# jcmgray/cotengra

Hardware: NVIDIA H100
Metric: sycamore_n53_m20_sliced_contract_tflops (higher is better)
Workload: dtype c128 (f64 arithmetic)

## Files before the change

### cotengra_b200/_lib.py

```python

from __future__ import annotations

import ctypes as C
import os

from . import lowering

_HERE = os.path.dirname(os.path.abspath(__file__))
LIB_PATH = os.path.join(_HERE, "libctgb200.so")

EXPORTS = (
    "ctgb_abi_version",
    "ctgb_desc_words",
    "ctgb_single_desc_words",
    "ctgb_last_error",
    "ctgb_device_info",
    "ctgb_contract_pair",
    "ctgb_reduce_single",
    "ctgb_plan_create",
    "ctgb_plan_set_chunk_desc",
    "ctgb_plan_set_scale_slots",
    "ctgb_plan_set_accumulator",
    "ctgb_plan_destroy",
    "ctgb_plan_workspace_bytes",
    "ctgb_plan_launches_per_slice",
    "ctgb_plan_strip_modes",
    "ctgb_plan_execute",
    "ctgb_plan_execute_host",
    "ctgb_launch_count",
    "ctgb_tensor_map_launches",
    "ctgb_plan_profile",
    "ctgb_plan_profile_read",
    "ctgb_probe_fp64_peaks",
    "ctgb_tc05_launch_config",
    "ctgb_dmmastream_launch_config",
)
TC05_LAUNCH_FIELDS = ("b_stat", "nb", "sa", "grid", "smem", "tm_rank", "bulk", "chunk_steps", "chunks")
DMMASTREAM_LAUNCH_FIELDS = ("nj", "rows", "grid")


class CtgbTensor(C.Structure):
    _fields_ = [
        ("kind", C.c_int32),
        ("input_index", C.c_int32),
        ("offset", C.c_int64),
        ("nbytes", C.c_int64),
        ("n_sliced", C.c_int32),
        ("slice_pos", C.POINTER(C.c_int32)),
        ("slice_stride", C.POINTER(C.c_int64)),
    ]
# ... 52 lines not shown
        if not hasattr(lib, name):
            raise ImportError(f"{LIB_PATH} does not export {name}")
    lib.ctgb_last_error.restype = C.c_char_p
    lib.ctgb_launch_count.restype = C.c_int64
    lib.ctgb_tensor_map_launches.restype = C.c_int64
    lib.ctgb_plan_workspace_bytes.restype = C.c_size_t
    lib.ctgb_plan_workspace_bytes.argtypes = [C.c_void_p]
    lib.ctgb_plan_launches_per_slice.restype = C.c_int64
    lib.ctgb_plan_launches_per_slice.argtypes = [C.c_void_p]
    lib.ctgb_plan_strip_modes.argtypes = [C.c_void_p, C.POINTER(C.c_int32), C.POINTER(C.c_int32), C.c_int]
    lib.ctgb_device_info.argtypes = [
        C.POINTER(C.c_int), C.POINTER(C.c_int), C.POINTER(C.c_int), C.POINTER(C.c_size_t)
    ]
    lib.ctgb_contract_pair.argtypes = [C.c_void_p] * 5
    lib.ctgb_reduce_single.argtypes = [C.c_void_p] * 4
    lib.ctgb_plan_create.argtypes = [C.POINTER(CtgbPlanDesc), C.POINTER(C.c_void_p)]
    lib.ctgb_plan_set_chunk_desc.argtypes = [C.c_void_p, C.c_void_p]
    lib.ctgb_plan_set_scale_slots.argtypes = [C.c_void_p, C.POINTER(C.c_int32), C.POINTER(C.c_int32), C.c_int]
    lib.ctgb_plan_set_accumulator.argtypes = [C.c_void_p, C.c_int32]
    lib.ctgb_plan_destroy.argtypes = [C.c_void_p]
    lib.ctgb_plan_destroy.restype = None
    lib.ctgb_plan_execute.argtypes = [
        C.c_void_p, C.POINTER(C.c_void_p), C.c_void_p, C.c_void_p, C.c_void_p, C.POINTER(C.c_void_p),
        C.c_void_p, C.c_size_t, C.c_int64, C.c_int64, C.c_int64, C.c_void_p,
    ]
    lib.ctgb_plan_execute_host.argtypes = [
        C.c_void_p, C.POINTER(C.c_void_p), C.POINTER(C.c_int64), C.c_void_p,
        C.POINTER(C.c_double), C.c_void_p, C.c_size_t, C.c_int64, C.c_int64,
        C.c_int64, C.c_void_p,
    ]
# ... 62 lines not shown
```

### cotengra_b200/contract.py

```python

from __future__ import annotations

import ctypes as C
import functools
import math
import warnings

import numpy as np

from . import _lib, lowering
from .executor import ExecPlan, output_chunking
from .lowering import (
    build_pair_desc,
    build_single_desc,
    check_accumulate,
    check_precision,
    check_tensordot_shapes,
    classify_pair,
    classify_single,
    dtype_name,
    split_equation,
    tensordot_terms,
)
from .tree import TreeSpec
# ... 110 lines not shown
    ta, tb, to = tensordot_terms(axes, na, nb)
    return _run_pair(ta, a, tb, b, to, precision)


def implementation(precision="3xtf32"):
    if check_precision(precision) == "3xtf32":
        return (einsum, tensordot)
    return (functools.partial(einsum, precision=precision), functools.partial(tensordot, precision=precision))




class _Executor:

    def __init__(self, contractions, inputs, output, size_dict, sliced, dtype, strip_exponent=False, device=None,
                 vjp_max_bytes=None, precision="3xtf32", stripped_grad=False, accumulate="native", **plan_opts):
        torch = _torch()
        self._ir, self._plan_opts = contractions, plan_opts
        self._program, self._sliced = (contractions, inputs, output, size_dict), sliced
        self.device = torch.device("cuda", torch.cuda.current_device() if device is None else device)
        with torch.cuda.device(self.device):
            self.plan = ExecPlan(*self._program, sliced, dtype=dtype, strip_exponent=strip_exponent,
                                 precision=precision, accumulate=accumulate, **plan_opts).create()
        self.dtype = self.plan.dtype
        self.precision = precision
        self.accumulate = accumulate
        self.out_dtype = self.plan.acc_dtype
        self.strip_exponent = bool(strip_exponent)
        self.stripped_grad = bool(stripped_grad)
        self.vjp_max_bytes = vjp_max_bytes
        self._shapes = [tuple(size_dict[ix] for ix in term) for term in inputs]
        self._ws = None
        self._vjp_plans, self._vjp_ws = {}, None

    @property
    def nslices(self):
        return self.plan.nslices

# ... 120 lines not shown
    def __init__(self, tree, dtype="complex128", strip_exponent=False, device=None,
                 contractions=None, fuse=True, vjp_max_bytes=None, precision="3xtf32", stripped_grad=False,
                 accumulate="native", **plan_opts):
        check_precision(precision, dtype)
        check_accumulate(accumulate)
        self.spec = spec = tree if isinstance(tree, TreeSpec) else TreeSpec.from_cotengra(tree)
        self.exec_spec, self.fusion = spec, {"changed": False}
        if fuse and contractions is None:
            from .fusion import fuse_stems

            opts = fuse if isinstance(fuse, dict) else {}
            self.exec_spec, self.fusion = fuse_stems(spec, dtype_name(dtype), **opts)
        ir = self.exec_spec.contractions() if contractions is None else contractions
        super().__init__(ir, spec.inputs, spec.output, spec.size_dict, spec.sliced, dtype,
                         strip_exponent=strip_exponent, device=device, vjp_max_bytes=vjp_max_bytes,
                         precision=precision, stripped_grad=stripped_grad, accumulate=accumulate, **plan_opts)
        self._ref_work = None

    @property
    def reference_work(self):
        if self._ref_work is None:
            if self.fusion.get("changed"):
                from .fusion import tree_work

                self._ref_work = tree_work(self.spec)
            else:
                self._ref_work = (self.plan.macs_per_slice, self.plan.macs_invariant,
                                  self.plan.elements_per_slice)
        return self._ref_work

    def __call__(self, arrays, **kw):
# ... 411 lines not shown
```

### cotengra_b200/csrc/ctg_b200.cu

```cuda
#include <cuda.h>
#include <cuda_runtime.h>
#include <stdint.h>
#include <stdio.h>
#include <stdlib.h>
#include <string.h>

#include <algorithm>
#include <atomic>
#include <type_traits>
#include <string>
#include <vector>

#include "../../include/ctg_b200.h"
#include "gett_desc.h"
#include "gett_kernels.cuh"
#include "probe.cuh"

using namespace ctgb;

namespace {

thread_local std::string g_err;
std::atomic<int64_t> g_launches{0};

// ... 237 lines not shown
  const bool strip = desc_stripped(h);
  const double2 *a = (const double2*)A, *b = (const double2*)B;
  double2* c = (double2*)C;
  const unsigned blocks = (unsigned)lc.blocks;
  switch (lc.nj) {
    case 1: dmmastream_launch<1, 4>(strip, blocks, d, a, b, c, st); break;
    case 2: dmmastream_launch<2, 4>(strip, blocks, d, a, b, c, st); break;
    case 4: dmmastream_launch<4, 4>(strip, blocks, d, a, b, c, st); break;
    default: dmmastream_launch<8, 2>(strip, blocks, d, a, b, c, st); break;
  }
  g_launches.fetch_add(1, std::memory_order_relaxed);
  CUDA_TRY(cudaGetLastError());
  return CTGB_OK;
}

std::atomic<int64_t> g_tmap_launches{0};

struct Tc05Box {
  int nb = 0;
  struct Dim { uint64_t ext, stride; } dim[8];
};
int tc05_tensor_map_box(const int64_t* h, uint64_t a_addr, Tc05Box& bx) {
  if (a_addr & 15u) return 0;
  auto& box = bx.dim;
  int& nb = bx.nb;
  nb = 0;
  const int n_lda = (int)h[W_NLDA];
  for (int i = 0; i < n_lda; ++i) {
    const uint64_t ext = (uint64_t)h[OFF_LDA + 4 * i], st = (uint64_t)h[OFF_LDA + 4 * i + 1];
    if (h[OFF_LDA + 4 * i + 1] <= 0) return 0;
// ... 236 lines not shown
             : launch_gett_policy<T, Tf32Policy<T, __VA_ARGS__>>(h, d, A, B, C, st)
      case VAR_DMMA_128x64: CTGB_TF32(4, 2, 2, 4, 16, 3);
      case VAR_DMMA_64x128: CTGB_TF32(2, 4, 2, 4, 16, 3);
      case VAR_DMMA_256x32: CTGB_TF32(8, 1, 2, 4, 8, 3);
      case VAR_DMMA_256x16: CTGB_TF32(8, 1, 2, 2, 8, 3);
      case VAR_TF32_32x32: CTGB_TF32(2, 2, 1, 2, 16, 4);
#undef CTGB_TF32
      default: break;
    }
  }
  return fail(CTGB_E_VALUE, "unknown kernel variant for this dtype");
}

int launch_gett(const int64_t* h, const int64_t* d, const void* A, const void* B, void* C, cudaStream_t st) {
  if (h[W_MAGIC] != DESC_MAGIC) return fail(CTGB_E_VALUE, "bad pair descriptor magic");
  switch ((int)h[W_DTYPE]) {
    case CTGB_F32: return launch_gett_typed<float>(h, d, A, B, C, st);
    case CTGB_F64: return launch_gett_typed<double>(h, d, A, B, C, st);
    case CTGB_C64: return launch_gett_typed<float2>(h, d, A, B, C, st);
    case CTGB_C128: return launch_gett_typed<double2>(h, d, A, B, C, st);
  }
  return fail(CTGB_E_VALUE, "bad dtype");
}

template <typename T>
int launch_single_typed(const int64_t* h, const int64_t* d, const void* X, void* out, cudaStream_t st) {
  long long n = h[S_OUT_ELEMS];
  if (n <= 0) return CTGB_OK;
  const long long cap = (long long)(devinfo().ok ? devinfo().sms : 132) * 16;
  long long blocks = (n + 255) / 256;
// ... 373 lines not shown
  cudaFree(sink);
  return rc;
}

int ctgb_contract_pair(const int64_t* desc, const void* A, const void* B, void* C, void* stream) {
  if (!desc) return fail(CTGB_E_VALUE, "null descriptor");
  cudaStream_t st = (cudaStream_t)stream;
  int64_t* d = nullptr;
  CUDA_TRY(cudaMallocAsync((void**)&d, DESC_WORDS * sizeof(int64_t), st));
  CUDA_TRY(cudaMemcpyAsync(d, desc, DESC_WORDS * sizeof(int64_t), cudaMemcpyHostToDevice, st));
  int rc = launch_gett(desc, d, A, B, C, st);
  cudaFreeAsync(d, st);
  return rc;
}

int ctgb_reduce_single(const int64_t* desc, const void* X, void* out, void* stream) {
  if (!desc) return fail(CTGB_E_VALUE, "null descriptor");
  cudaStream_t st = (cudaStream_t)stream;
  int64_t* d = nullptr;
  CUDA_TRY(cudaMallocAsync((void**)&d, SDESC_WORDS * sizeof(int64_t), st));
  CUDA_TRY(cudaMemcpyAsync(d, desc, SDESC_WORDS * sizeof(int64_t), cudaMemcpyHostToDevice, st));
  int rc = launch_single(desc, d, X, out, st);
  cudaFreeAsync(d, st);
  return rc;
}

int ctgb_plan_create(const ctgb_plan_desc* pd, ctgb_plan** out) {
  if (!pd || !out) return fail(CTGB_E_VALUE, "null argument");
  const size_t es = elem_size(pd->dtype);
  if (es == 0) return fail(CTGB_E_VALUE, "bad dtype");
// ... 14 lines not shown
    const ctgb_node& n = pd->nodes[i];
    auto& q = p->nodes[i];
    q.kind = n.kind;
    q.a = n.a;
    q.b = n.b;
    q.c = n.c;
    q.phase = n.phase;
    q.zero_fill = n.zero_fill;
    q.is_root = n.is_root;
    const int words = n.kind == 0 ? (int)DESC_WORDS : (int)SDESC_WORDS;
    const int64_t magic = n.kind == 0 ? DESC_MAGIC : SDESC_MAGIC;
    if (n.kind < 0 || n.kind > 1 || !n.desc || n.desc[0] != magic) return refuse("bad node descriptor");
    if (n.phase < 0 || n.phase > 3) return refuse("bad node phase");
    auto bad = [&](int t) { return t < 0 || t >= pd->n_tensors; };
    if (bad(n.a) || bad(n.c) || (n.kind == 0 && bad(n.b))) return refuse("node refers to a missing tensor");
    p->backward |= n.phase >= 2;
    if (n.is_root) p->root = i;
    if (n.kind == 0 && (n.desc[W_FLAGS] & FLAG_WIDE_C)) {
      if (!n.is_root || pd->strip_exponent) return refuse("a wide C belongs to the root of an unstripped plan");
      p->wide_desc = true;
    }
    q.desc_off = p->descs.size();
    p->descs.insert(p->descs.end(), n.desc, n.desc + words);
    q.c_elems = p->tensors[n.c].nbytes / (int64_t)es;
    if (pd->strip_exponent && n.kind == 0) {
      const int64_t* w = n.desc;
      q.measure_after = w[W_SPLITK] > 1 || w[W_VARIANT] == VAR_DOTSTREAM || w[W_VARIANT] == VAR_DOTSTREAM4;
      q.measure_after |= w[W_VARIANT] == VAR_KRED;
      q.measure_after |= (w[W_VARIANT] == VAR_TC05_128x64 || w[W_VARIANT] == VAR_TC05_128x32 ||
                          w[W_VARIANT] == VAR_TC05_128x16) &&
// ... 216 lines not shown
        char* base = under(tb);
        if (int r = scale_copy(p->dtype, base, p->d_bscale, tb.nbytes / (int64_t)es, p->d_factors + n.fa,
                               p->d_factors + n.fb, st))
          return r;
        B = p->d_bscale + (B - base);
      }
      if (n.prescale_a) {
        const ctgb_plan::Tensor& ta = p->tensors[n.a];
        char* base = under(ta);
        const double* one = p->d_factors + p->tensors.size() + 1;
        if (int r = scale_copy(p->dtype, base, p->d_bscale, ta.nbytes / (int64_t)es, p->d_factors + n.fa,
                               n.fb >= 0 ? p->d_factors + n.fb : one, st))
          return r;
        A = p->d_bscale + (A - base);
      }
      if (int r = launch_node(n.kind, h, d, A, B, C, st)) return r;
      if (n.measure_after) {
        if (int r = absmax_into(p->dtype, C, n.c_elems, (unsigned long long*)(p->d_factors + n.c), st)) return r;
      }
      if (p->profile) cudaEventRecord(p->ev1[ni], st);
    }
    return CTGB_OK;
  };

  if (p->strip_exponent && p->n_inv_slots > 0) {
    reset_slots_kernel<<<1, 256, 0, st>>>(p->d_factors, p->d_slot_lists + p->n_var_slots, p->n_inv_slots);
    g_launches.fetch_add(1, std::memory_order_relaxed);
  }
  if ((rc = run_phase(0, 0))) return rc;
  if (p->strip_exponent) {
    sum_log_kernel<<<1, 256, 0, st>>>(p->d_factors, p->d_slot_lists + p->n_var_slots, p->n_inv_slots, d_inv_exp,
// ... 106 lines not shown
```

### cotengra_b200/csrc/gett_desc.h

```cpp
#pragma once
#include <stdint.h>

namespace ctgb {

constexpr int MAX_T = 12;
constexpr int MAX_G = 40;
constexpr int MAX_GB = 12;
constexpr int MAX_LD = 24;

enum : int {
  W_MAGIC = 0,
  W_DTYPE = 1,
  W_NTM = 2, W_NTN = 3, W_NTK = 4,
  W_NGM = 5, W_NGN = 6, W_NGK = 7, W_NGB = 8,
  W_MTA = 9, W_NTA = 10, W_KTA = 11,
  W_TILES_M = 12, W_TILES_N = 13, W_TILES_B = 14, W_STEPS_K = 15,
  W_SPLITK = 16,
  W_PGM = 17, W_MFULL = 18, W_MTEXT = 19, W_MW = 20,
  W_PGN = 21, W_NFULL = 22, W_NTEXT = 23, W_NW = 24,
  W_PGK = 25, W_KFULL = 26, W_KTEXT = 27, W_KW = 28,
  W_NLDA = 29, W_NLDB = 30,
  W_FLAGS = 31,
  W_VARIANT = 32,
  W_CELEMS = 33,
// ... 25 lines not shown
  VAR_DMMA_256x32 = 4,
  VAR_DMMA_256x16 = 5,
  VAR_ROW_128x8 = 6,
  VAR_ROW_256x4 = 7,
  VAR_ROWSTREAM = 8,
  VAR_TC05_128x64 = 9,
  VAR_TC05_128x32 = 10,
  VAR_TC05_128x16 = 11,
  VAR_DMMA3M_128x32 = 12,
  VAR_DMMA3M_256x16 = 13,
  VAR_DOTSTREAM = 15,
  VAR_DMMASTREAM = 14,
  VAR_DOTSTREAM4 = 16,
  VAR_ROWSTREAM_K = 19,
  VAR_DMMA_32x32 = 18,
  VAR_TF32_32x32 = 20
};

constexpr int MAX_S = 40;
enum : int {
  S_MAGIC = 0, S_DTYPE = 1, S_NO = 2, S_NS = 3, S_OUT_ELEMS = 4, S_SUM_ELEMS = 5,
  S_FLAGS = 6,
  S_HDR = 8,
  OFF_SO = S_HDR,
  OFF_SS = OFF_SO + MAX_S * 3,
  SDESC_WORDS = OFF_SS + MAX_S * 2
};
constexpr int64_t SDESC_MAGIC = 0x43544742'53303031LL;

}
```

### cotengra_b200/csrc/gett_kernels.cuh

```cuda
#pragma once
#include <cuda_runtime.h>
#include <math_constants.h>
#include <stdint.h>

#include <type_traits>

#include "gett_desc.h"

namespace ctgb {

__device__ __forceinline__ void mac(float& c, float a, float b) { c = fmaf(a, b, c); }
__device__ __forceinline__ void mac(double& c, double a, double b) { c = fma(a, b, c); }
__device__ __forceinline__ void mac(float2& c, float2 a, float2 b) {
  c.x = fmaf(a.x, b.x, c.x);
  c.x = fmaf(-a.y, b.y, c.x);
  c.y = fmaf(a.x, b.y, c.y);
  c.y = fmaf(a.y, b.x, c.y);
}
__device__ __forceinline__ void mac(double2& c, double2 a, double2 b) {
  c.x = fma(a.x, b.x, c.x);
  c.x = fma(-a.y, b.y, c.x);
  c.y = fma(a.x, b.y, c.y);
  c.y = fma(a.y, b.x, c.y);
}
// ... 515 lines not shown
            store(r, c + 1, make_double2(acc.re[i][j][1], acc.im[i][j][1]));
          }
        } else {
          store(r, c, acc.re[i][j][0]);
          store(r, c + 1, acc.re[i][j][1]);
        }
      }
  }
};

#include "tf32_policy.cuh"
#include "stream_rows.cuh"
#include "rowstream.cuh"
#include "dmmastream.cuh"
#include "dotstream.cuh"
#include "tc05_policy.cuh"
#include "gett_ws.cuh"
#include "tc05_kernel.cuh"

template <typename T>
__global__ void single_kernel(const int64_t* __restrict__ D, const T* __restrict__ X, T* __restrict__ out) {
  const int n_o = (int)D[S_NO], n_s = (int)D[S_NS];
  const long long out_elems = D[S_OUT_ELEMS], sum_elems = D[S_SUM_ELEMS];
  const bool accumulate = (D[S_FLAGS] & 1) != 0;
  for (long long o = blockIdx.x * (long long)blockDim.x + threadIdx.x; o < out_elems;
       o += (long long)gridDim.x * blockDim.x) {
    long long e = o, xo = 0, oo = 0;
    for (int d = 0; d < n_o; ++d) {
      const int64_t* L = D + OFF_SO + d * 3;
      long long dig = e % L[0];
// ... 202 lines not shown
```

### cotengra_b200/executor.py

```python

from __future__ import annotations

import ctypes as C
import math

import numpy as np

from . import _lib, lowering
from .lowering import (
    DTYPE_CODES,
    DTYPE_SIZES,
    accumulator_dtype,
    build_pair_desc,
    build_single_desc,
    check_precision,
    check_tensordot_shapes,
    classify_pair,
    classify_single,
    dtype_name,
    row_major_strides,
    split_equation,
    tensordot_terms,
)

# ... 84 lines not shown
        self.last_use = -1


def layout(sched, reserve=0):
    for t in _slots(sched):
        t.first_use, t.last_use, t.offset = None, -1, 0
    zero_pos = sched.index(None) if None in sched else 0
    end_loop = max((pos for pos, nd in enumerate(sched) if nd is not None and nd["phase"] in LOOP_PHASES),
                   default=zero_pos)
    for pos, nd in enumerate(sched):
        if nd is None:
            continue
        c = nd["c"]
        if c.first_use is None:
            c.first_use = zero_pos if c.kind == K_HACC else pos
        for s in (nd["a"], nd["b"]):
            if s is None:
                continue
            s.last_use = max(s.last_use, pos)
            if s.kind == K_PERSISTENT and nd["phase"] in LOOP_PHASES:
                s.last_use = max(s.last_use, end_loop)
    persistent, scratch = _Arena(), _Arena()
    reserved = persistent.alloc(reserve) if reserve else -1
    arena = {K_SCRATCH: scratch, K_PERSISTENT: persistent, K_HACC: persistent}
    allocs, releases = {}, {}
    for t in _slots(sched):
        if t.kind in arena:
            t.last_use = max(t.last_use, t.first_use)
            allocs.setdefault(t.first_use, []).append(t)
            releases.setdefault(t.last_use, []).append(t)
    for pos in range(len(sched)):
        for t in allocs.get(pos, ()):
            t.offset = arena[t.kind].alloc(t.nbytes)
        for t in releases.get(pos, ()):
            arena[t.kind].release(t.offset, t.nbytes)
    return _align(scratch.peak), _align(persistent.peak), reserved


def _slots(sched):
    return list(dict.fromkeys(t for nd in sched if nd is not None for t in (nd["a"], nd["b"], nd["c"])
                              if t is not None))


class _DevicePlan:

    handle = None
    strip_exponent = False
    cotangent_offset = -1
    acc_dtype = None
    _chunk_words = None
    scale_slots = None

    def _marshal(self):
        keep = self._keep = []
        slot = {id(t): i for i, t in enumerate(self.tensors)}
        ct = (_lib.CtgbTensor * max(len(self.tensors), 1))()
        for i, t in enumerate(self.tensors):
            ct[i].kind = t.kind
            ct[i].input_index = t.input_index
            ct[i].offset = t.offset
            ct[i].nbytes = t.nbytes
            ct[i].n_sliced = len(t.slice_pos)
            if t.slice_pos:
                pos = (C.c_int32 * len(t.slice_pos))(*t.slice_pos)
                st = (C.c_int64 * len(t.slice_stride))(*t.slice_stride)
                keep += [pos, st]
                ct[i].slice_pos = C.cast(pos, C.POINTER(C.c_int32))
                ct[i].slice_stride = C.cast(st, C.POINTER(C.c_int64))
        cn = (_lib.CtgbNode * max(len(self.nodes), 1))()
        for i, nd in enumerate(self.nodes):
            words = np.ascontiguousarray(nd["words"], dtype=np.int64)
            keep.append(words)
            cn[i].kind = nd["kind"]
            cn[i].a = slot[id(nd["a"])]
            cn[i].b = slot[id(nd["b"])] if nd["b"] is not None else -1
            cn[i].c = slot[id(nd["c"])]
            cn[i].phase = nd["phase"]
            cn[i].zero_fill = int(nd.get("zero_fill", False))
            cn[i].is_root = int(nd.get("root", False))
            cn[i].desc = words.ctypes.data_as(C.POINTER(C.c_int64))
        ns = len(self.sliced)
        radix = (C.c_int64 * max(ns, 1))(*[s for _i, s, _p in self.sliced])
        proj = (C.c_int64 * max(ns, 1))(*[(-1 if p is None else p) for _i, _s, p in self.sliced])
        ostr = (C.c_int64 * max(ns, 1))(*self.slice_out_stride)
        keep += [ct, cn, radix, proj, ostr]
        pd = self._pd = _lib.CtgbPlanDesc()
# ... 45 lines not shown
        pre, after = (C.c_int32 * n)(), (C.c_int32 * n)()
        _lib.check(_lib.load().ctgb_plan_strip_modes(self.handle, pre, after, n))
        return [(int(a), int(b)) for a, b in zip(pre, after)]

    def __del__(self):
        try:
            self.destroy()
        except Exception:
            pass


class ExecPlan(_DevicePlan):

    def __init__(self, contractions, inputs, output, size_dict, sliced=(), dtype="complex128",
                 strip_exponent=False, hoist=True, allow_dmma=True, sm_count=None,
                 variant=None, precision="3xtf32", accumulate="native"):
        self.dtype = dtype_name(dtype)
        self.precision = check_precision(precision, self.dtype)
        self.esize = DTYPE_SIZES[self.dtype]
        self.acc_dtype = accumulator_dtype(self.dtype, accumulate)
        self.wide = self.acc_dtype != self.dtype
        self.contractions = tuple(contractions)
        self.inputs = [tuple(t) for t in inputs]
        self.output = tuple(output)
        self.size_dict = dict(size_dict)
        self.sliced = [(i, int(s), None if p is None else int(p)) for i, s, p in sliced]
        self.strip_exponent = bool(strip_exponent)
        if sm_count is None:
            try:
                sm_count = _lib.device_info()["sm_count"]
            except Exception:
                sm_count = 132
        self.sm_count = sm_count
        self._build(hoist, allow_dmma, variant)

    def _build(self, hoist, allow_dmma, variant):
        sliced_pos = {ind: j for j, (ind, _s, _p) in enumerate(self.sliced)}
        nslices = math.prod(s for _i, s, p in self.sliced if p is None)
        self.nslices = nslices
        real_slicing = bool(self.sliced)
        hoist = hoist and real_slicing

        def out_ext(ix):
            if ix in sliced_pos and self.sliced[sliced_pos[ix]][2] is not None:
                return 1
            return self.size_dict[ix]

        self.out_shape = tuple(out_ext(ix) for ix in self.output)
# ... 69 lines not shown
                                                    c_dense_elems=dense, variant=variant,
                                                    precision=self.precision, wide_c=wide_c)

            if is_root and self.wide and not self.strip_exponent:
                direct = lower(True)[2].variant in lowering.DOTSTREAM_VARIANTS
                dims, dense, plan = lower(direct, wide_c=direct)
            else:
                dims, dense, plan = lower(is_root and direct)
            if is_root:
                self._check_root_shape(dims.out_shape)
            acc = is_root and direct
            dst = _Slot(dims.out_shape, row_major_strides(dims.out_shape), K_SCRATCH,
                        max(math.prod(dims.out_shape), 1) * self.esize, variant=A.variant or Bt.variant)
            a, b = (Bt, A) if plan.swapped else (A, Bt)
            nodes.append(dict(kind=0, a=a, b=b, c=dst, words=plan.words, root=is_root, plan=plan,
                              sizes=plan.sizes, dims=dims, acc=acc, dense=dense))
            tensors.append(dst)
            cur[p] = dst

        if not nodes:
            raise ValueError("empty contraction program")
        self.root_direct = direct
        if direct:
            nodes[-1]["c"].kind = K_OUTPUT
        for nd in nodes:
            srcs = [nd["a"]] + ([nd["b"]] if nd["b"] is not None else [])
            nd["invariant"] = bool(hoist and not nd["root"] and not any(s.variant for s in srcs))
            nd["phase"] = PHASE_INV_FWD if nd["invariant"] else PHASE_VAR_FWD
            if nd["invariant"]:
                nd["c"].kind = K_PERSISTENT
            else:
                nd["c"].variant = True
        order = [nd for nd in nodes if nd["invariant"]] + [nd for nd in nodes if not nd["invariant"]]
        for pos, nd in enumerate(order):
            nd["pos"] = pos
        self.workspace_bytes, self.persistent_bytes, _ = layout(order)
        self.nodes = nodes
        self.n_variant_nodes = sum(1 for nd in nodes if not nd["invariant"])

        self.macs_per_slice = 0
        self.macs_invariant = 0
        self.elements_per_slice = 0
        for nd in nodes:
            if nd["kind"] != 0:
                continue
            Bn, M, N, K = nd["sizes"]
            macs = Bn * M * N * K
            el = math.prod(nd["a"].shape) + math.prod(nd["b"].shape) + math.prod(nd["c"].shape)
            if nd["invariant"]:
                self.macs_invariant += macs
            else:
                self.macs_per_slice += macs
                self.elements_per_slice += el

        self.tensors = tensors
        self._marshal()
        if not direct:
            rs = self.root_shape
            dense = row_major_strides(rs)
            odims = [[e, sx, so] for e, sx, so in zip(rs, dense, root_strides) if e != 1]
            self._chunk_words = build_single_desc(odims, [], self.dtype)

    def _check_root_shape(self, shape):
        if tuple(shape) != tuple(self.root_shape):
            raise ValueError(
                f"contraction program produces shape {tuple(shape)}, "
                f"tree output expects {tuple(self.root_shape)}"
            )

    def host_staging_bytes(self):
        extra = _align(self.total_bytes) - self.total_bytes
        for n in self.input_nbytes:
            extra += _align(n)
        return extra + _align(self.out_elements * DTYPE_SIZES[self.acc_dtype]) + 512

    def execute(self, input_ptrs, out_ptr, exp_ptr, ws_ptr, ws_bytes, begin, step, count, stream=0):
# ... 24 lines not shown
```

### cotengra_b200/lowering.py

```python

from __future__ import annotations

import math
from collections import Counter, namedtuple
from dataclasses import dataclass, field

import numpy as np

MAX_T, MAX_G, MAX_GB, MAX_LD = 12, 40, 12, 24
(W_MAGIC, W_DTYPE, W_NTM, W_NTN, W_NTK, W_NGM, W_NGN, W_NGK, W_NGB, W_MTA,
 W_NTA, W_KTA, W_TILES_M, W_TILES_N, W_TILES_B, W_STEPS_K, W_SPLITK, W_PGM,
 W_MFULL, W_MTEXT, W_MW, W_PGN, W_NFULL, W_NTEXT, W_NW, W_PGK, W_KFULL,
 W_KTEXT, W_KW, W_NLDA, W_NLDB, W_FLAGS, W_VARIANT, W_CELEMS, W_RUNA, W_LBOPAD) = range(36)
W_HDR = 40
OFF_TM = W_HDR
OFF_TN = OFF_TM + MAX_T * 3
OFF_TK = OFF_TN + MAX_T * 3
OFF_GM = OFF_TK + MAX_T * 3
OFF_GN = OFF_GM + MAX_G * 4
OFF_GK = OFF_GN + MAX_G * 4
OFF_GB = OFF_GK + MAX_G * 4
OFF_LDA = OFF_GB + MAX_GB * 5
OFF_LDB = OFF_LDA + MAX_LD * 4
DESC_WORDS = OFF_LDB + MAX_LD * 4
DESC_MAGIC = 0x4354474232303031

MAX_S = 40
S_MAGIC, S_DTYPE, S_NO, S_NS, S_OUT_ELEMS, S_SUM_ELEMS, S_FLAGS = range(7)
S_HDR = 8
OFF_SO = S_HDR
OFF_SS = OFF_SO + MAX_S * 3
SDESC_WORDS = OFF_SS + MAX_S * 2
SDESC_MAGIC = 0x4354474253303031

VAR_SIMT_64x64, VAR_KRED, VAR_DMMA_128x64, VAR_DMMA_64x128, VAR_DMMA_256x32 = 0, 1, 2, 3, 4
VAR_DMMA_256x16, VAR_ROW_128x8, VAR_ROW_256x4, VAR_ROWSTREAM = 5, 6, 7, 8
VAR_TC05_128x64, VAR_TC05_128x32, VAR_TC05_128x16 = 9, 10, 11
VAR_DMMA3M_128x32, VAR_DMMA3M_256x16, VAR_DMMASTREAM, VAR_DOTSTREAM, VAR_DOTSTREAM4 = 12, 13, 14, 15, 16
VAR_DMMA_32x32, VAR_ROWSTREAM_K, VAR_TF32_32x32 = 18, 19, 20
DMMASTREAM_KMAX, DMMASTREAM_WIDE_N, DMMASTREAM_WIDE_KMAX = 64, 64, 32


def dmmastream_fits(N, K):
    return (N <= 32 and K <= DMMASTREAM_KMAX) or (N <= DMMASTREAM_WIDE_N and K <= DMMASTREAM_WIDE_KMAX)


DMMASTREAM_MAX_N = 32


TC05_VARIANTS = (VAR_TC05_128x64, VAR_TC05_128x32, VAR_TC05_128x16)
TC05_MAX_K = 16384
TC05_CHUNK_STEPS = 16
VARIANT_TILES = {
    VAR_SIMT_64x64: (64, 64, 8),
# ... 519 lines not shown
    W[W_SPLITK] = splitk
    for base, p in ((W_PGM, t.pm), (W_PGN, t.pn), (W_PGK, t.pk)):
        W[base:base + 4] = (-1, 0, 0, 0) if p is None else p
    W[W_NLDA], W[W_NLDB] = len(t.lda), len(t.ldb)
    W[W_FLAGS], W[W_VARIANT], W[W_CELEMS], W[W_RUNA], W[W_LBOPAD] = flags, t.variant, int(c_dense_elems), run_a, lbopad
    for off, rows, width in ((OFF_TM, t.tm, 3), (OFF_TN, t.tn, 3), (OFF_TK, t.tk, 3), (OFF_GM, t.gm, 4),
                             (OFF_GN, t.gn, 4), (OFF_GK, t.gk, 4), (OFF_GB, t.gb, 5), (OFF_LDA, t.lda, 4),
                             (OFF_LDB, t.ldb, 4)):
        for i, r in enumerate(rows):
            W[off + i * width: off + (i + 1) * width] = r
    return W




def classify_single(term, shape, out, out_strides=None, strides_x=None):
    term, out = tuple(term), tuple(out)
    shape = tuple(map(int, shape))
    if len(term) != len(shape):
        raise ValueError(f"Term '{term}' does not match shape {shape}.")
    sx = row_major_strides(shape) if strides_x is None else list(strides_x)
    ext, st_x, order = {}, {}, []
    for ix, d, s in zip(term, shape, sx):
        if ix not in order:
            order.append(ix)
        if ext.setdefault(ix, d) != d:
            raise ValueError(f"Index {ix} has mismatched sizes {ext[ix]} and {d}.")
        st_x[ix] = st_x.get(ix, 0) + s
    for ix in out:
        if ix not in ext:
# ... 42 lines not shown
```

### include/ctg_b200.h

```cpp
#ifndef CTG_B200_H
#define CTG_B200_H

#include <stddef.h>
#include <stdint.h>

#ifdef __cplusplus
extern "C" {
#endif

#define CTGB_ABI_VERSION 2

enum {
  CTGB_F32 = 0,
  CTGB_F64 = 1,
  CTGB_C64 = 2,
  CTGB_C128 = 3
};

enum {
  CTGB_OK = 0,
  CTGB_E_VALUE = 1,
  CTGB_E_NOTIMPL = 2,
  CTGB_E_CUDA = 3,
  CTGB_E_MEMORY = 4
};

int ctgb_abi_version(void);
int ctgb_desc_words(void);
int ctgb_single_desc_words(void);
const char* ctgb_last_error(void);

int ctgb_device_info(int* sm_count, int* cc_major, int* cc_minor,
                     size_t* smem_optin_bytes);

int ctgb_contract_pair(const int64_t* desc, const void* A, const void* B,
                       void* C, void* stream);

int ctgb_reduce_single(const int64_t* desc, const void* X, void* out,
                       void* stream);


typedef struct ctgb_plan ctgb_plan;

typedef struct {
  int32_t kind;
  int32_t input_index;
  int64_t offset;
  int64_t nbytes;
  int32_t n_sliced;
  const int32_t* slice_pos;
  const int64_t* slice_stride;
// ... 70 lines not shown
```

Before: 23.35.

## Fuse penultimate pair contraction into root contraction with three-operand absorb kernel

Adds a complex128 DMMA kernel that folds the last two pairwise contractions into one launch. It computes the small intermediate X from the big and small operands on the fly in registers and multiplies it straight into V, so the large intermediate tensor is never written to or read back from global memory. The executor rewrites the final node pair when the shapes fit the kernel's fixed limits and it is enabled by default when fuse is set. The tradeoff is a cross-warp shared-memory reduction followed by atomic adds into the output, recomputation of X for each column chunk, and narrow applicability.

```diff
diff --git a/cotengra_b200/_lib.py b/cotengra_b200/_lib.py
--- a/cotengra_b200/_lib.py
+++ b/cotengra_b200/_lib.py
@@ -34,6 +34,7 @@
     "ctgb_probe_fp64_peaks",
     "ctgb_tc05_launch_config",
     "ctgb_dmmastream_launch_config",
+    "ctgb_absorb_root",
 )
 TC05_LAUNCH_FIELDS = ("b_stat", "nb", "sa", "grid", "smem", "tm_rank", "bulk", "chunk_steps", "chunks")
 DMMASTREAM_LAUNCH_FIELDS = ("nj", "rows", "grid")
@@ -116,6 +117,7 @@
     ]
     lib.ctgb_contract_pair.argtypes = [C.c_void_p] * 5
     lib.ctgb_reduce_single.argtypes = [C.c_void_p] * 4
+    lib.ctgb_absorb_root.argtypes = [C.c_void_p] * 6
     lib.ctgb_plan_create.argtypes = [C.POINTER(CtgbPlanDesc), C.POINTER(C.c_void_p)]
     lib.ctgb_plan_set_chunk_desc.argtypes = [C.c_void_p, C.c_void_p]
     lib.ctgb_plan_set_scale_slots.argtypes = [C.c_void_p, C.POINTER(C.c_int32), C.POINTER(C.c_int32), C.c_int]
diff --git a/cotengra_b200/contract.py b/cotengra_b200/contract.py
--- a/cotengra_b200/contract.py
+++ b/cotengra_b200/contract.py
@@ -148,14 +148,16 @@
 class _Executor:
 
     def __init__(self, contractions, inputs, output, size_dict, sliced, dtype, strip_exponent=False, device=None,
-                 vjp_max_bytes=None, precision="3xtf32", stripped_grad=False, accumulate="native", **plan_opts):
+                 vjp_max_bytes=None, precision="3xtf32", stripped_grad=False, accumulate="native", absorb_root=False,
+                 **plan_opts):
         torch = _torch()
         self._ir, self._plan_opts = contractions, plan_opts
         self._program, self._sliced = (contractions, inputs, output, size_dict), sliced
         self.device = torch.device("cuda", torch.cuda.current_device() if device is None else device)
         with torch.cuda.device(self.device):
             self.plan = ExecPlan(*self._program, sliced, dtype=dtype, strip_exponent=strip_exponent,
-                                 precision=precision, accumulate=accumulate, **plan_opts).create()
+                                 precision=precision, accumulate=accumulate, absorb_root=absorb_root,
+                                 **plan_opts).create()
         self.dtype = self.plan.dtype
         self.precision = precision
         self.accumulate = accumulate
@@ -306,7 +308,8 @@
         ir = self.exec_spec.contractions() if contractions is None else contractions
         super().__init__(ir, spec.inputs, spec.output, spec.size_dict, spec.sliced, dtype,
                          strip_exponent=strip_exponent, device=device, vjp_max_bytes=vjp_max_bytes,
-                         precision=precision, stripped_grad=stripped_grad, accumulate=accumulate, **plan_opts)
+                         precision=precision, stripped_grad=stripped_grad, accumulate=accumulate,
+                         absorb_root=bool(fuse) and contractions is None, **plan_opts)
         self._ref_work = None
 
     @property
diff --git a/cotengra_b200/csrc/absorbdot.cuh b/cotengra_b200/csrc/absorbdot.cuh
--- /dev/null
+++ b/cotengra_b200/csrc/absorbdot.cuh
@@ -0,0 +1,172 @@
+#pragma once
+
+constexpr int AB_STAGES = 4;
+constexpr int AB_THREADS = 256;
+constexpr int AB_VSTAGE = 2 * 32 * 32;
+constexpr int AB_ASTAGE = 2 * 32 * 16;
+constexpr size_t AB_SMEM = (size_t)(128 * 16 + AB_STAGES * (AB_VSTAGE + AB_ASTAGE)) * sizeof(double2);
+
+__device__ __forceinline__ double ab_neg(double x) { return __longlong_as_double(__double_as_longlong(x) ^ (1ll << 63)); }
+
+__global__ void __launch_bounds__(AB_THREADS, 1)
+absorbdot_kernel(const int64_t* __restrict__ D, const double2* __restrict__ A, const double2* __restrict__ Bs,
+                 const double2* __restrict__ V, double2* __restrict__ C) {
+  extern __shared__ __align__(16) double2 ab_smem[];
+  double2* sB = ab_smem;
+  double2* sV = sB + 128 * 16;
+  double2* sA = sV + AB_STAGES * AB_VSTAGE;
+  __shared__ long long t_ma[32], t_mc[32], t_nv[32], t_cv[128], t_ka[16];
+
+  const int tid = threadIdx.x, lane = tid & 31, warp = tid >> 5;
+  const int N = (int)D[AB_N], K = (int)D[AB_K], CC = (int)D[AB_C], CCP = (int)D[AB_CCP], KL = (int)D[AB_KL];
+  const int NG = (int)D[AB_NG];
+  const long long kla = D[AB_KLA], klv = D[AB_KLV];
+  for (int i = tid; i < 32; i += AB_THREADS) {
+    t_ma[i] = D[AB_TMA + i];
+    t_mc[i] = D[AB_TMC + i];
+    t_nv[i] = D[AB_TNV + i];
+  }
+  for (int i = tid; i < 128; i += AB_THREADS) t_cv[i] = D[AB_TCV + i];
+  for (int i = tid; i < 16; i += AB_THREADS) t_ka[i] = D[AB_TKA + i];
+  for (int i = tid; i < 128 * 16; i += AB_THREADS) {
+    const int c = i >> 4, k = i & 15;
+    const long long cb = D[AB_TCB + c];
+    const bool ok = cb >= 0 && k < K;
+    cp_async_zfill<16>(sB + c * 16 + (k ^ ((c & 1) << 2)), ok ? Bs + D[AB_TKB + k] + cb : Bs, ok);
+  }
+  __syncthreads();
+
+  const unsigned long long U = (unsigned long long)D[AB_UNITS];
+  const unsigned u0 = (unsigned)(U * blockIdx.x / gridDim.x), u1 = (unsigned)(U * (blockIdx.x + 1) / gridDim.x);
+  const int nq = CCP >> 5;
+  const long long nstage = (long long)(u1 - u0) * nq;
+
+  unsigned g_ext = 1, g_div = 1;
+  long long g_sa = 0, g_sv = 0;
+  if (lane < NG) {
+    g_ext = (unsigned)D[AB_G + lane * 4];
+    g_div = (unsigned)D[AB_G + lane * 4 + 1];
+    g_sa = D[AB_G + lane * 4 + 2];
+    g_sv = D[AB_G + lane * 4 + 3];
+  }
+  auto unit_base = [&](unsigned u, long long& oa, long long& ov) {
+    const long long dgt = (long long)((u / g_div) % g_ext);
+    long long a = dgt * g_sa, v = dgt * g_sv;
+#pragma unroll
+    for (int o = 16; o > 0; o >>= 1) {
+      a += __shfl_xor_sync(0xffffffffu, a, o);
+      v += __shfl_xor_sync(0xffffffffu, v, o);
+    }
+    oa = a;
+    ov = v;
+  };
+
+  unsigned lu = u0;
+  int lq = 0;
+  long long la = 0, lv = 0;
+  if (nstage > 0) unit_base(lu, la, lv);
+  long long issued = 0;
+  auto issue = [&]() {
+    if (issued < nstage) {
+      const int slot = (int)(issued % AB_STAGES);
+      double2* dv = sV + slot * AB_VSTAGE;
+      double2* da = sA + slot * AB_ASTAGE;
+#pragma unroll
+      for (int j = 0; j < 8; ++j) {
+        const int e = j * AB_THREADS + tid, cq = e & 31, kl = (e >> 5) & 1, n = e >> 6, c = lq * 32 + cq;
+        const bool ok = kl < KL && n < N && c < CC;
+        cp_async_zfill<16>(dv + (kl * 32 + n) * 32 + (cq ^ (n & 1)), ok ? V + lv + kl * klv + t_nv[n] + t_cv[c] : V, ok);
+      }
+#pragma unroll
+      for (int j = 0; j < 4; ++j) {
+        const int e = j * AB_THREADS + tid, k = e & 15, kl = (e >> 4) & 1, m = e >> 5;
+        const bool ok = k < K && kl < KL && t_mc[m] >= 0;
+        cp_async_zfill<16>(da + (kl * 32 + m) * 16 + (k ^ ((m & 1) << 2)), ok ? A + la + kl * kla + t_ka[k] + t_ma[m] : A,
+                           ok);
+      }
+      ++issued;
+      if (++lq == nq) {
+        lq = 0;
+        ++lu;
+        if (issued < nstage) unit_base(lu, la, lv);
+      }
+    }
+    cp_async_commit();
+  };
+#pragma unroll 1
+  for (int s = 0; s < AB_STAGES - 1; ++s) issue();
+
+  const int g = lane >> 2, t = lane & 3;
+  const int wmh = warp >> 2, wcb = warp & 3;
+  int bofs[2];
+#pragma unroll
+  for (int i = 0; i < 2; ++i) bofs[i] = (int)D[AB_TBCK + 2 * wmh + i] * CCP * 16;
+  double Rr[4][2][2], Ri[4][2][2];
+#pragma unroll
+  for (int nb = 0; nb < 4; ++nb)
+#pragma unroll
+    for (int i = 0; i < 2; ++i) Rr[nb][i][0] = Rr[nb][i][1] = Ri[nb][i][0] = Ri[nb][i][1] = 0.0;
+
+#pragma unroll 1
+  for (long long s = 0; s < nstage; ++s) {
+    cp_async_wait<AB_STAGES - 2>();
+    __syncthreads();
+    issue();
+    const int slot = (int)(s % AB_STAGES), q = (int)(s % nq);
+    if (q * 32 + wcb * 8 >= CC) continue;
+    const double2* vb = sB + (q * 32 + wcb * 8 + g) * 16;
+#pragma unroll
+    for (int kl = 0; kl < 2; ++kl) {
+      if (kl >= KL) break;
+      const double2* va = sA + slot * AB_ASTAGE + (kl * 32 + wmh * 16) * 16;
+      const double2* vv = sV + slot * AB_VSTAGE + kl * 32 * 32;
+      double Xr[2][2], Xi[2][2];
+#pragma unroll
+      for (int i = 0; i < 2; ++i) Xr[i][0] = Xr[i][1] = Xi[i][0] = Xi[i][1] = 0.0;
+#pragma unroll
+      for (int ks = 0; ks < 4; ++ks) {
+        const int kk = (ks * 4 + t) ^ ((g & 1) << 2);
+#pragma unroll
+        for (int i = 0; i < 2; ++i) {
+          const double2 b = vb[bofs[i] + kk];
+          const double2 a = va[(i * 8 + g) * 16 + kk];
+          dmma16x8x4(Xr[i], Xi[i], a.x, a.y, b.x);
+          dmma16x8x4(Xr[i], Xi[i], ab_neg(a.y), a.x, b.y);
+        }
+      }
+#pragma unroll
+      for (int p = 0; p < 2; ++p) {
+#pragma unroll
+        for (int nb = 0; nb < 4; ++nb) {
+          const double2 v = vv[(nb * 8 + g) * 32 + ((wcb * 8 + 2 * t + p) ^ (g & 1))];
+          const double nvi = ab_neg(v.y);
+#pragma unroll
+          for (int i = 0; i < 2; ++i) {
+            dmma16x8x4(Rr[nb][i], Ri[nb][i], v.x, v.y, Xr[i][p]);
+            dmma16x8x4(Rr[nb][i], Ri[nb][i], nvi, v.x, Xi[i][p]);
+          }
+        }
+      }
+    }
+  }
+  cp_async_wait<0>();
+  __syncthreads();
+
+  double2* red = sV;
+#pragma unroll
+  for (int nb = 0; nb < 4; ++nb)
+#pragma unroll
+    for (int i = 0; i < 2; ++i)
+#pragma unroll
+      for (int e = 0; e < 2; ++e)
+        red[wcb * 1024 + ((2 * wmh + i) * 8 + 2 * t + e) * 32 + nb * 8 + g] = make_double2(Rr[nb][i][e], Ri[nb][i][e]);
+  __syncthreads();
+  for (int i = tid; i < 1024; i += AB_THREADS) {
+    const int m = i >> 5, n = i & 31;
+    if (t_mc[m] < 0 || n >= N) continue;
+    double2 sum = red[i];
+#pragma unroll
+    for (int w = 1; w < 4; ++w) sum = add_of(sum, red[w * 1024 + i]);
+    atomic_add_of(C + t_mc[m] + D[AB_TNC + n], sum);
+  }
+}
diff --git a/cotengra_b200/csrc/ctg_b200.cu b/cotengra_b200/csrc/ctg_b200.cu
--- a/cotengra_b200/csrc/ctg_b200.cu
+++ b/cotengra_b200/csrc/ctg_b200.cu
@@ -275,6 +275,32 @@
   return CTGB_OK;
 }
 
+int launch_absorb_root(const int64_t* h, const int64_t* d, const void* A, const void* Bs, const void* V, void* C,
+                       cudaStream_t st) {
+  if (h[W_DTYPE] != CTGB_C128) return fail(CTGB_E_VALUE, "the absorb-root kernel is complex128 only");
+  if (h[AB_M] < 1 || h[AB_M] > 32 || h[AB_N] < 1 || h[AB_N] > 32 || h[AB_K] < 1 || h[AB_K] > 16 || h[AB_C] < 1 ||
+      h[AB_C] > h[AB_CCP] || h[AB_CCP] % 32 || h[AB_CCP] > 128 || (h[AB_KL] != 1 && h[AB_KL] != 2) || h[AB_NG] < 0 || h[AB_NG] > AB_MAXG || h[AB_UNITS] < 1 || h[AB_UNITS] >= (1ll << 32) ||
+      h[AB_GRID] < 1 || h[AB_GRID] > h[AB_UNITS] || h[AB_GRID] > (1 << 20))
+    return fail(CTGB_E_VALUE, "absorb-root descriptor out of range");
+  for (int mb = 0; mb < 4; ++mb)
+    if (h[AB_TBCK + mb] < 0 || (h[AB_TBCK + mb] + 1) * h[AB_CCP] > 128)
+      return fail(CTGB_E_VALUE, "absorb-root descriptor out of range");
+  if (!(h[W_FLAGS] & 1)) {
+    if (h[W_CELEMS] <= 0) return fail(CTGB_E_VALUE, "absorb-root into a strided C needs accumulate");
+    CUDA_TRY(cudaMemsetAsync(C, 0, (size_t)h[W_CELEMS] * sizeof(double2), st));
+  }
+  static bool attr = false;
+  if (!attr) {
+    CUDA_TRY(cudaFuncSetAttribute(absorbdot_kernel, cudaFuncAttributeMaxDynamicSharedMemorySize, (int)AB_SMEM));
+    attr = true;
+  }
+  absorbdot_kernel<<<(unsigned)h[AB_GRID], AB_THREADS, AB_SMEM, st>>>(d, (const double2*)A, (const double2*)Bs,
+                                                                      (const double2*)V, (double2*)C);
+  g_launches.fetch_add(1, std::memory_order_relaxed);
+  CUDA_TRY(cudaGetLastError());
+  return CTGB_OK;
+}
+
 std::atomic<int64_t> g_tmap_launches{0};
 
 struct Tc05Box {
@@ -541,6 +567,7 @@
 
 int launch_gett(const int64_t* h, const int64_t* d, const void* A, const void* B, void* C, cudaStream_t st) {
   if (h[W_MAGIC] != DESC_MAGIC) return fail(CTGB_E_VALUE, "bad pair descriptor magic");
+  if (h[W_VARIANT] == VAR_ABSORB_ROOT) return fail(CTGB_E_VALUE, "an absorb-root node has three operands (ctgb_absorb_root)");
   switch ((int)h[W_DTYPE]) {
     case CTGB_F32: return launch_gett_typed<float>(h, d, A, B, C, st);
     case CTGB_F64: return launch_gett_typed<double>(h, d, A, B, C, st);
@@ -944,6 +971,18 @@
   return rc;
 }
 
+int ctgb_absorb_root(const int64_t* desc, const void* A, const void* Bs, const void* V, void* C, void* stream) {
+  if (!desc || desc[0] != DESC_MAGIC || desc[W_VARIANT] != VAR_ABSORB_ROOT)
+    return fail(CTGB_E_VALUE, "not an absorb-root descriptor");
+  cudaStream_t st = (cudaStream_t)stream;
+  int64_t* d = nullptr;
+  CUDA_TRY(cudaMallocAsync((void**)&d, DESC_WORDS * sizeof(int64_t), st));
+  CUDA_TRY(cudaMemcpyAsync(d, desc, DESC_WORDS * sizeof(int64_t), cudaMemcpyHostToDevice, st));
+  int rc = launch_absorb_root(desc, d, A, Bs, V, C, st);
+  cudaFreeAsync(d, st);
+  return rc;
+}
+
 int ctgb_reduce_single(const int64_t* desc, const void* X, void* out, void* stream) {
   if (!desc) return fail(CTGB_E_VALUE, "null descriptor");
   cudaStream_t st = (cudaStream_t)stream;
@@ -988,6 +1027,10 @@
     if (n.phase < 0 || n.phase > 3) return refuse("bad node phase");
     auto bad = [&](int t) { return t < 0 || t >= pd->n_tensors; };
     if (bad(n.a) || bad(n.c) || (n.kind == 0 && bad(n.b))) return refuse("node refers to a missing tensor");
+    if (n.kind == 0 && n.desc[W_VARIANT] == VAR_ABSORB_ROOT) {
+      if (bad((int)n.desc[AB_BS_SLOT])) return refuse("node refers to a missing tensor");
+      if (pd->strip_exponent) return refuse("an absorb-root node runs in unstripped plans only");
+    }
     p->backward |= n.phase >= 2;
     if (n.is_root) p->root = i;
     if (n.kind == 0 && (n.desc[W_FLAGS] & FLAG_WIDE_C)) {
@@ -1234,7 +1277,11 @@
           return r;
         A = p->d_bscale + (A - base);
       }
-      if (int r = launch_node(n.kind, h, d, A, B, C, st)) return r;
+      if (n.kind == 0 && h[W_VARIANT] == VAR_ABSORB_ROOT) {
+        if (int r = launch_absorb_root(h, d, A, resolve((int)h[AB_BS_SLOT], out_off), B, C, st)) return r;
+      } else if (int r = launch_node(n.kind, h, d, A, B, C, st)) {
+        return r;
+      }
       if (n.measure_after) {
         if (int r = absmax_into(p->dtype, C, n.c_elems, (unsigned long long*)(p->d_factors + n.c), st)) return r;
       }
diff --git a/cotengra_b200/csrc/gett_desc.h b/cotengra_b200/csrc/gett_desc.h
--- a/cotengra_b200/csrc/gett_desc.h
+++ b/cotengra_b200/csrc/gett_desc.h
@@ -63,8 +63,33 @@
   VAR_DOTSTREAM4 = 16,
   VAR_ROWSTREAM_K = 19,
   VAR_DMMA_32x32 = 18,
-  VAR_TF32_32x32 = 20
+  VAR_TF32_32x32 = 20,
+  VAR_ABSORB_ROOT = 21
 };
+
+constexpr int AB_MAXG = 32;
+enum : int {
+  AB_M = 2, AB_N = 3, AB_K = 4, AB_C = 5,
+  AB_KL = 6,
+  AB_NG = 7,
+  AB_UNITS = 8,
+  AB_KLA = 9, AB_KLV = 10,
+  AB_GRID = 11,
+  AB_BS_SLOT = 12,
+  AB_CCP = 13,
+  AB_TMA = W_HDR,
+  AB_TMC = AB_TMA + 32,
+  AB_TNV = AB_TMC + 32,
+  AB_TNC = AB_TNV + 32,
+  AB_TKA = AB_TNC + 32,
+  AB_TKB = AB_TKA + 16,
+  AB_TCB = AB_TKB + 16,
+  AB_TCV = AB_TCB + 128,
+  AB_G = AB_TCV + 128,
+  AB_TBCK = AB_G + AB_MAXG * 4,
+  AB_WORDS = AB_TBCK + 4
+};
+static_assert(AB_WORDS <= DESC_WORDS, "absorb-root words fit a pair descriptor");
 
 constexpr int MAX_S = 40;
 enum : int {
diff --git a/cotengra_b200/csrc/gett_kernels.cuh b/cotengra_b200/csrc/gett_kernels.cuh
--- a/cotengra_b200/csrc/gett_kernels.cuh
+++ b/cotengra_b200/csrc/gett_kernels.cuh
@@ -553,6 +553,7 @@
 #include "rowstream.cuh"
 #include "dmmastream.cuh"
 #include "dotstream.cuh"
+#include "absorbdot.cuh"
 #include "tc05_policy.cuh"
 #include "gett_ws.cuh"
 #include "tc05_kernel.cuh"
diff --git a/cotengra_b200/executor.py b/cotengra_b200/executor.py
--- a/cotengra_b200/executor.py
+++ b/cotengra_b200/executor.py
@@ -122,7 +122,7 @@
         c = nd["c"]
         if c.first_use is None:
             c.first_use = zero_pos if c.kind == K_HACC else pos
-        for s in (nd["a"], nd["b"]):
+        for s in (nd["a"], nd["b"], nd.get("d")):
             if s is None:
                 continue
             s.last_use = max(s.last_use, pos)
@@ -146,7 +146,7 @@
 
 
 def _slots(sched):
-    return list(dict.fromkeys(t for nd in sched if nd is not None for t in (nd["a"], nd["b"], nd["c"])
+    return list(dict.fromkeys(t for nd in sched if nd is not None for t in (nd["a"], nd["b"], nd.get("d"), nd["c"])
                               if t is not None))
 
 
@@ -177,7 +177,9 @@
                 ct[i].slice_stride = C.cast(st, C.POINTER(C.c_int64))
         cn = (_lib.CtgbNode * max(len(self.nodes), 1))()
         for i, nd in enumerate(self.nodes):
-            words = np.ascontiguousarray(nd["words"], dtype=np.int64)
+            words = np.array(nd["words"], dtype=np.int64)
+            if nd.get("d") is not None:
+                words[lowering.AB_BS_SLOT] = slot[id(nd["d"])]
             keep.append(words)
             cn[i].kind = nd["kind"]
             cn[i].a = slot[id(nd["a"])]
@@ -253,7 +255,7 @@
 
     def __init__(self, contractions, inputs, output, size_dict, sliced=(), dtype="complex128",
                  strip_exponent=False, hoist=True, allow_dmma=True, sm_count=None,
-                 variant=None, precision="3xtf32", accumulate="native"):
+                 variant=None, precision="3xtf32", accumulate="native", absorb_root=False):
         self.dtype = dtype_name(dtype)
         self.precision = check_precision(precision, self.dtype)
         self.esize = DTYPE_SIZES[self.dtype]
@@ -271,6 +273,8 @@
             except Exception:
                 sm_count = 132
         self.sm_count = sm_count
+        self.absorb_root = bool(absorb_root) and self.dtype == "complex128" and not self.strip_exponent \
+            and variant is None
         self._build(hoist, allow_dmma, variant)
 
     def _build(self, hoist, allow_dmma, variant):
@@ -370,9 +374,11 @@
                         max(math.prod(dims.out_shape), 1) * self.esize, variant=A.variant or Bt.variant)
             a, b = (Bt, A) if plan.swapped else (A, Bt)
             nodes.append(dict(kind=0, a=a, b=b, c=dst, words=plan.words, root=is_root, plan=plan,
-                              sizes=plan.sizes, dims=dims, acc=acc, dense=dense))
+                              sizes=plan.sizes, dims=dims, acc=acc, dense=dense, terms=(A, Bt)))
             tensors.append(dst)
             cur[p] = dst
+            if self.absorb_root:
+                self._absorb(nodes, tensors)
 
         if not nodes:
             raise ValueError("empty contraction program")
@@ -380,7 +386,7 @@
         if direct:
             nodes[-1]["c"].kind = K_OUTPUT
         for nd in nodes:
-            srcs = [nd["a"]] + ([nd["b"]] if nd["b"] is not None else [])
+            srcs = [t for t in (nd["a"], nd["b"], nd.get("d")) if t is not None]
             nd["invariant"] = bool(hoist and not nd["root"] and not any(s.variant for s in srcs))
             nd["phase"] = PHASE_INV_FWD if nd["invariant"] else PHASE_VAR_FWD
             if nd["invariant"]:
@@ -400,9 +406,8 @@
         for nd in nodes:
             if nd["kind"] != 0:
                 continue
-            Bn, M, N, K = nd["sizes"]
-            macs = Bn * M * N * K
-            el = math.prod(nd["a"].shape) + math.prod(nd["b"].shape) + math.prod(nd["c"].shape)
+            macs = nd["plan"].macs if nd.get("d") is not None else math.prod(nd["sizes"])
+            el = sum(math.prod(nd[x].shape) for x in ("a", "b", "d", "c") if nd.get(x) is not None)
             if nd["invariant"]:
                 self.macs_invariant += macs
             else:
@@ -416,6 +421,26 @@
             dense = row_major_strides(rs)
             odims = [[e, sx, so] for e, sx, so in zip(rs, dense, root_strides) if e != 1]
             self._chunk_words = build_single_desc(odims, [], self.dtype)
+
+    def _absorb(self, nodes, tensors):
+        if len(nodes) < 2:
+            return
+        P, R = nodes[-2], nodes[-1]
+        if P["kind"] != 0 or R["kind"] != 0 or P.get("d") is not None or R["plan"].variant != lowering.VAR_DMMA_32x32:
+            return
+        X = P["c"]
+        if X not in R["terms"]:
+            return
+        ab = lowering.build_absorb_desc(P["dims"], R["dims"], R["terms"][0] is X, accumulate=R["acc"],
+                                        sm_count=self.sm_count, c_dense_elems=R["dense"])
+        if ab is None:
+            return
+        pa, pb = P["terms"]
+        small, big = (pa, pb) if ab.small_is_a else (pb, pa)
+        V = R["terms"][1] if R["terms"][0] is X else R["terms"][0]
+        tensors.remove(X)
+        nodes[-2:] = [dict(kind=0, a=big, b=V, d=small, c=R["c"], words=ab.words, root=R["root"], plan=ab,
+                           sizes=ab.sizes, dims=None, acc=R["acc"], dense=R["dense"], terms=None)]
 
     def _check_root_shape(self, shape):
         if tuple(shape) != tuple(self.root_shape):
diff --git a/cotengra_b200/lowering.py b/cotengra_b200/lowering.py
--- a/cotengra_b200/lowering.py
+++ b/cotengra_b200/lowering.py
@@ -38,6 +38,7 @@
 VAR_TC05_128x64, VAR_TC05_128x32, VAR_TC05_128x16 = 9, 10, 11
 VAR_DMMA3M_128x32, VAR_DMMA3M_256x16, VAR_DMMASTREAM, VAR_DOTSTREAM, VAR_DOTSTREAM4 = 12, 13, 14, 15, 16
 VAR_DMMA_32x32, VAR_ROWSTREAM_K, VAR_TF32_32x32 = 18, 19, 20
+VAR_ABSORB_ROOT = 21
 DMMASTREAM_KMAX, DMMASTREAM_WIDE_N, DMMASTREAM_WIDE_KMAX = 64, 64, 32
 
 
@@ -587,6 +588,112 @@
 
 
 
+AB_M, AB_N, AB_K, AB_C, AB_KL, AB_NG, AB_UNITS, AB_KLA, AB_KLV, AB_GRID, AB_BS_SLOT, AB_CCP = range(2, 14)
+AB_MAXG = 32
+AB_TMA = W_HDR
+AB_TMC, AB_TNV, AB_TNC = AB_TMA + 32, AB_TMA + 64, AB_TMA + 96
+AB_TKA = AB_TMA + 128
+AB_TKB = AB_TKA + 16
+AB_TCB = AB_TKB + 16
+AB_TCV = AB_TCB + 128
+AB_G = AB_TCV + 128
+AB_TBCK = AB_G + AB_MAXG * 4
+
+
+@dataclass
+class AbsorbPlan:
+
+    words: np.ndarray
+    small_is_a: bool
+    sizes: tuple
+    macs: int
+    variant: int = VAR_ABSORB_ROOT
+    swapped: bool = False
+    splitk: int = 1
+    tiles: int = 1
+
+
+def _enum(dims, cols):
+    out = [[0] for _ in cols]
+    for d in dims:
+        out = [[o + i * d[c] for i in range(d[0]) for o in lst] for lst, c in zip(out, cols)]
+    return out
+
+
+def build_absorb_desc(dp: PairDims, dr: PairDims, x_is_a, accumulate=False, sm_count=132, c_dense_elems=0):
+    if dp.batch or dr.batch:
+        return None
+    xi = 1 if x_is_a else 2
+    vi = 3 - xi
+    r_keep = {d[xi]: (d[0], d[3]) for d in (dr.m if x_is_a else dr.n)}
+    v_keep = [[d[0], d[vi], d[3]] for d in (dr.n if x_is_a else dr.m)]
+    r_con = {d[xi]: (d[0], d[vi]) for d in dr.k}
+    if len(r_con) != len(dr.k) or len(r_keep) != len(dr.m if x_is_a else dr.n):
+        return None
+    for small_is_a in (False, True):
+        small = dp.m if small_is_a else dp.n
+        big = dp.n if small_is_a else dp.m
+        bi, si = (2, 1) if small_is_a else (1, 2)
+        xdims = {d[3]: d for d in small + big}
+        if not small or len(xdims) != len(small) + len(big) or set(xdims) != set(r_keep) | set(r_con):
+            continue
+        if any(xdims[x][0] != (r_keep.get(x) or r_con[x])[0] for x in xdims):
+            continue
+        small_x = {d[3] for d in small}
+        rows = [[d[0], d[bi], r_keep[d[3]][1]] for d in big if d[3] in r_keep]
+        ck = [[d[0], d[si], r_keep[d[3]][1]] for d in small if d[3] in r_keep]
+        cc = sorted(([d[0], d[si], r_con[d[3]][1]] for d in small if d[3] in r_con), key=lambda d: d[2])
+        kprime = [[d[0], d[bi], r_con[d[3]][1]] for d in big if d[3] in r_con]
+        MX, CK = math.prod(d[0] for d in rows), math.prod(d[0] for d in ck)
+        N, K, CC = math.prod(d[0] for d in v_keep), math.prod(d[0] for d in dp.k), math.prod(d[0] for d in cc)
+        CCP = -(-CC // 32) * 32
+        rows_per = 8 if CK > 1 else 32
+        if MX > rows_per or CK * rows_per > 32 or N > 32 or K > 16 or CK * CCP > 128 or not small_x:
+            return None
+        kl = min(kprime, key=lambda d: d[2], default=None)
+        if kl is not None and kl[0] == 2:
+            kprime.remove(kl)
+        else:
+            kl = [1, 0, 0]
+        grid = sorted(kprime, key=lambda d: (d[1], d[2]))
+        if len(grid) > AB_MAXG:
+            return None
+        units = math.prod(d[0] for d in grid)
+        w = np.zeros(DESC_WORDS, dtype=np.int64)
+        w[0], w[1] = DESC_MAGIC, DTYPE_CODES["complex128"]
+        w[AB_M], w[AB_N], w[AB_K], w[AB_C], w[AB_CCP], w[AB_KL] = CK * rows_per if CK > 1 else MX, N, K, CC, CCP, kl[0]
+        w[AB_NG], w[AB_UNITS], w[AB_KLA], w[AB_KLV] = len(grid), units, kl[1], kl[2]
+        w[AB_GRID] = min(units, sm_count)
+        w[AB_BS_SLOT] = -1
+        w[W_FLAGS] = int(bool(accumulate))
+        w[W_VARIANT] = VAR_ABSORB_ROOT
+        w[W_CELEMS] = c_dense_elems
+        ra, rc = _enum(rows, (1, 2))
+        ckb, ckc = _enum(ck, (1, 2))
+        ma, mc = [-1] * 32, [-1] * 32
+        for j, (ob, oc) in enumerate(zip(ckb, ckc)):
+            for r, (a, c) in enumerate(zip(ra, rc)):
+                ma[j * rows_per + r], mc[j * rows_per + r] = a, c + oc
+        tbck = [min(mb * 8 // rows_per, CK - 1) for mb in range(4)]
+        nv, nc = _enum(v_keep, (1, 2))
+        ka, kb = _enum([[d[0], d[bi], d[si]] for d in dp.k], (1, 2))
+        cb, cv = _enum(cc, (1, 2))
+        tcb = [-1] * 128
+        for j, ob in enumerate(ckb):
+            tcb[j * CCP:j * CCP + CC] = [ob + o for o in cb]
+        for off, vals in ((AB_TMA, ma), (AB_TMC, mc), (AB_TNV, nv), (AB_TNC, nc), (AB_TKA, ka), (AB_TKB, kb),
+                          (AB_TCB, tcb), (AB_TCV, cv), (AB_TBCK, tbck)):
+            w[off:off + len(vals)] = vals
+        div = 1
+        for j, (e, sa, sv) in enumerate(grid):
+            w[AB_G + 4 * j:AB_G + 4 * j + 4] = (e, div, sa, sv)
+            div *= e
+        kp = units * kl[0]
+        M = MX * CK
+        return AbsorbPlan(w, small_is_a, (1, M, N, kp * CC), MX * kp * K * CC * CK + M * N * kp * CC)
+    return None
+
+
 def classify_single(term, shape, out, out_strides=None, strides_x=None):
     term, out = tuple(term), tuple(out)
     shape = tuple(map(int, shape))
diff --git a/include/ctg_b200.h b/include/ctg_b200.h
--- a/include/ctg_b200.h
+++ b/include/ctg_b200.h
@@ -35,6 +35,9 @@
 
 int ctgb_contract_pair(const int64_t* desc, const void* A, const void* B,
                        void* C, void* stream);
+
+int ctgb_absorb_root(const int64_t* desc, const void* A, const void* Bs,
+                     const void* V, void* C, void* stream);
 
 int ctgb_reduce_single(const int64_t* desc, const void* X, void* out,
                        void* stream);
```

Result: faster. 24.19 (median of 6 runs) (+3.6%).
